# Vanlightly/vsr-tlaplus

Measured on AMD Instinct MI355X. Metric: distinct states/sec (whole node) + time-to-first-violation, VSR 3-replica, higher is better.
Workload: dtype u64

## Files before the change

vsr_tlaplus_amd/csrc/vsr_deep.hpp:

```cpp
#pragma once

namespace {

typedef DeepLevelRec DeepLevel;

struct Slicer {
  u64 cap_n, cap_w, g1, stride;
  u64 cap_c = ~(u64)0;
  double yield_n = 0, yield_w = 0;
  u64 worst() const {
    const u64 sz = std::min<u64>(std::min<u64>(cap_n / (4 * g1), cap_w / (4 * g1 * stride)), cap_c);
    return std::max<u64>(128, sz & ~(u64)127);
  }
  u64 next() const {
    if (yield_n <= 0) return worst();
    const double sz = std::min((double)cap_n / (3.0 * std::max(yield_n, 1e-3)), (double)cap_w / (3.0 * std::max(yield_w, 1e-3)));
    return std::max<u64>(worst(), std::min<u64>(cap_c, std::max<u64>(128, (u64)std::min(sz, 1e15) & ~(u64)127)));
  }
  void expect(double per_n, double per_w) { yield_n = std::max(yield_n, per_n); yield_w = std::max(yield_w, per_w); }
  void observe(u64 n_src, u64 n_out, u64 w_out) {
    if (!n_src) return;
    yield_n = std::max(yield_n, (double)n_out / (double)n_src);
    yield_w = std::max(yield_w, (double)w_out / (double)n_src);
  }
};

struct DeepRun;
struct DeepIo {
  void* ctx = nullptr;
  int world = 1;
  u64 cand_cap = 0;
  int (*pass)(void* ctx, const u64* sw, const u64* so, u64 n, u64 p_off, int level, int mode, u64 bag, const PassDst* dst) = nullptr;
  int (*any)(void* ctx, u64* flag) = nullptr;
  int (*reduce)(void* ctx, DeepRun* R) = nullptr;
  int (*resolve)(void* ctx, DeepRun* R) = nullptr;
};

struct DeepRun {
  vsrmc_checker* c;
  const DeepIo* io = nullptr;
  int base;
  int last_regen;
  bool insert;
  vsrmc_level_info ins, prb;
  u64 viol_ins = ~(u64)0;
  u32 mask_ins = 0, mask_prb = 0;
  std::vector<u64> bad;
  u64 launches = 0, n_slices = 0, n_subs = 0;
  u64* d_sum = nullptr;
  bool rebase = false;
  u64* d_cnt = nullptr;
  u32* d_err = nullptr;
  int err = 0;
  int probed_level() const { return last_regen + (insert ? 2 : 1); }
};

void deep_free_scratch(vsrmc_checker* c) {
  for (PassDst& B : c->scratch) {
    if (B.words && B.own_words) (void)hipFree(B.words);
    if (B.off && B.own_index) (void)hipFree(B.off);
    if (B.fp && B.own_index) (void)hipFree(B.fp);
  }
  c->scratch.clear();
  c->scratch0 = PassDst();
  c->scratch_carved = false;
  c->scratch_buf = -1;
  c->scratch_front = 0;
}

int deep_plan_scratch(vsrmc_checker* c, int count, bool carve = true, u64 front = 0) {
  if (count < 0) count = 0;
  if (count > 400) return fail(VSRMC_E_REP, "deep search: more than 400 nested levels");
  const int nxt = c->cur ^ 1;
  if ((c->host_frontier >> nxt) & 1) carve = false;
  front = (front + 63) & ~(u64)63;
  const bool same_buf = !c->scratch_carved || c->scratch_buf == nxt;
  if ((size_t)count <= c->scratch.size() && c->scratch_front == front && same_buf && (c->scratch_carved == carve || (count == 0 && !carve))) return 0;
  deep_free_scratch(c);
  if (count == 0) return 0;
  size_t free_b = 0, total_b = 0;
  HIPCHK(hipMemGetInfo(&free_b, &total_b));
  const char* share_env = std::getenv("VSRMC_AUTOSIZE_SHARE");
  const double share = share_env ? std::max(1.0, std::atof(share_env)) : 1.0;
  const double reserve = std::max(0.0, (double)free_b - 1.0e9) / share;
  if (front >= c->words_cap(nxt)) carve = false;
  const double idle_w = (double)(c->words_cap(nxt) - (carve ? front : 0));
  const int with0 = front ? 0 : 1;
  const u64 floor_w = (u64)1 << 21;
  const double w_old = std::max((double)floor_w, std::min(idle_w / 4.0, reserve / (double)count / 9.34));
  const double cost_old = (with0 ? 1.0 / idle_w : 0.0) + (double)count / w_old;
  int best_n = 0;
  double best_s = 0;
  if (carve)
    for (int n_idle = 1; n_idle <= count + with0; n_idle++) {
      const double from_res = (double)(count + with0 - n_idle) * 9.34 + (double)(n_idle - with0) * 1.34;
      const double s = std::min(idle_w / (double)n_idle, from_res > 0 ? reserve / from_res : 1e30);
      if (s > best_s) { best_s = s; best_n = n_idle; }
    }
  const bool carved = carve && best_n >= 1 + with0 && best_s >= (double)floor_w && (double)(count + with0) / best_s < cost_old;
  const u64 wcap = carved ? (u64)best_s & ~(u64)63 : (u64)w_old;
  auto alloc_index = [&](PassDst& B) -> bool {
    B.cap = std::max<u64>((u64)1 << 15, B.words_cap / 12);
    return hipMalloc((void**)&B.off, (B.cap + 1) * 8) == hipSuccess && hipMalloc((void**)&B.fp, B.cap * 8) == hipSuccess;
  };
  bool ok = true;
  if (carved && with0) {
    c->scratch0.words = c->words[nxt]; c->scratch0.words_cap = wcap; c->scratch0.own_words = false;
    c->scratch0.off = c->off[nxt]; c->scratch0.fp = c->lvl_fp; c->scratch0.own_index = false;
    c->scratch0.cap = std::min<u64>(c->opt.frontier_states, std::max<u64>((u64)1 << 15, wcap / 12));
  }
  for (int k = 1; k <= count && ok; k++) {
    PassDst B;
    B.words_cap = wcap;
    if (carved && k - 1 + with0 < best_n) { B.words = c->words[nxt] + front + (u64)(k - 1 + with0) * wcap; B.own_words = false; }
    else ok = hipMalloc((void**)&B.words, B.words_cap * 8) == hipSuccess;
    ok = ok && alloc_index(B);
    c->scratch.push_back(B);
  }
  if (!ok) {
    (void)hipGetLastError();
    deep_free_scratch(c);
    return fail(VSRMC_E_HIP, "hipMalloc of a deep-search scratch buffer failed");
  }
  c->scratch_carved = carve;
  c->scratch_buf = nxt;
  c->scratch_front = front;
  return 0;
}

int deep_buffer(vsrmc_checker* c, int k, PassDst* out) {
  const int nxt = c->cur ^ 1;
  if (k == 0) {
    if (c->scratch0.words) { *out = c->scratch0; return 0; }
    out->words = c->words[nxt]; out->words_cap = c->words_cap(nxt); out->off = c->off[nxt]; out->fp = c->lvl_fp; out->cap = c->opt.frontier_states;
    return 0;
  }
  if ((size_t)k > c->scratch.size()) return fail(VSRMC_E_REP, "deep search: a nesting level without a planned scratch buffer");
  *out = c->scratch[(size_t)k - 1];
  return 0;
}

void deep_acc(vsrmc_level_info* t, const LevelCtl& h, double ms) {
  t->generated += h.generated;
  t->deadlocks += h.deadlocks;
  t->probes += h.probes;
  for (int a = 0; a < 16; a++) t->act_generated[a] += h.act_generated[a];
  t->expand_ms += ms;
}

int deep_run_pass(DeepRun& R, const u64* sw, const u64* so, u64 n, u64 p_off, int level, int mode, u64 bag, const PassDst* dst) {
  R.c->extra_launches = 0;
  if (R.io) return R.io->pass(R.io->ctx, sw, so, n, p_off, level, mode, bag, dst);
  return expand_pass(R.c, sw, so, n, p_off, level, mode, bag, dst);
}

void deep_claim_bits_alloc(vsrmc_checker* c, u64 src_max_bag) {
  if (c->claim_bits) { (void)hipFree(c->claim_bits); c->claim_bits = nullptr; }
  c->claim_w = c->claim_parents = 0;
  if (c->opt.world > 1 || !c->regen_bits_kernel || !c->insert_kernel) return;
  const Model& M = c->model.M;
  const u64 ords = (u64)M.m0 + std::min<u64>(src_max_bag, (u64)M.max_bag) * (u64)(M.R + 1) + 1;
  const u64 w = (ords + 31) / 32, bytes = c->n_frontier * w * 4;
  if (w > 8) return;
  size_t free_b = 0, total_b = 0;
  if (hipMemGetInfo(&free_b, &total_b) != hipSuccess || (double)bytes > 0.4 * (double)free_b) return;
  if (hipMalloc((void**)&c->claim_bits, std::max<u64>(bytes, 4)) != hipSuccess) { (void)hipGetLastError(); c->claim_bits = nullptr; return; }
  if (hipMemsetAsync(c->claim_bits, 0, std::max<u64>(bytes, 4), c->stream) != hipSuccess) { (void)hipFree(c->claim_bits); c->claim_bits = nullptr; return; }
  c->claim_w = w;
  c->claim_parents = c->n_frontier;
}
bool deep_more(DeepRun& R, bool mine, int* rc) {
  u64 f = (mine ? 1 : 0) | (R.err ? 2 : 0);
  if (R.io) *rc = R.io->any(R.io->ctx, &f);
  if (!*rc && f >= 2) *rc = R.err ? R.err : fail(VSRMC_E_STATE, "deep pass: another rank failed between two exchanges");
  return !*rc && (f & 1) != 0;
}
int deep_local_fail(DeepRun& R, int rc) {
  if (!R.io) return rc;
  if (!R.err) R.err = rc;
  return 0;
}
u64 deep_cand_bound(const DeepRun& R, u64 g1) {
  if (!R.io || R.io->world <= 1) return ~(u64)0;
  return std::max<u64>(128, (u64)(0.45 * (double)R.io->cand_cap * (double)R.io->world / (double)std::max<u64>(1, g1)) & ~(u64)127);
}

int deep_probe(DeepRun& R, const PassDst& B, u64 n, int lv, u64 bag) {
  vsrmc_checker* c = R.c;
  if (!n) return 0;
  c->expand_ms = 0;
  if (R.err) return 0;
  int rc = expand_pass(c, B.words, B.off, n, 0, lv + 1, MODE_PROBE, bag);
  R.launches += c->extra_launches;
  if (!rc && c->h.limit_unchecked) {
    R.prb.limit_rechecked += c->h.limit_unchecked;
    c->probe_all_actions = true;
    rc = expand_pass(c, B.words, B.off, n, 0, lv + 1, MODE_PROBE, bag);
    c->probe_all_actions = false;
    R.launches += 1 + c->extra_launches;
  }
  if (rc) return deep_local_fail(R, rc);
  R.launches++;
  deep_acc(&R.prb, c->h, c->expand_ms);
  if (c->h.n_pending) {
    R.mask_prb |= c->h.viol_mask;
    if (c->h.n_pending > c->opt.pending_entries || R.bad.size() / 2 + c->h.n_pending > ((u64)1 << 24))
      return deep_local_fail(R, fail(VSRMC_E_REP, "more violating successors in the probed level than the pending list holds (pending_entries)"));
    const size_t at = R.bad.size();
    R.bad.resize(at + 2 * c->h.n_pending);
    if (hipMemcpy(R.bad.data() + at, c->pending, 16 * c->h.n_pending, hipMemcpyDeviceToHost) != hipSuccess)
      return deep_local_fail(R, fail(VSRMC_E_HIP, "deep search: copy of the probe's candidates"));
  }
  return 0;
}

int deep_export(DeepRun& R, const PassDst& B, u64 part) {
  vsrmc_checker* c = R.c;
  if (!part) return 0;
  const int nxt = c->cur ^ 1;
  hipLaunchKernelGGL(k_export, dim3((unsigned)((part + 63) / 64)), dim3(64), 0, c->stream, (const u64*)B.words, B.off, B.fp, (u64)0, part,
                     c->words[nxt], c->scratch_front ? c->scratch_front : c->words_cap(nxt), c->off[nxt], c->lvl_fp, c->opt.frontier_states, R.d_cnt, R.d_err);
  if (hipGetLastError() != hipSuccess || hipStreamSynchronize(c->stream) != hipSuccess) return fail(VSRMC_E_HIP, "deep search: k_export (re-basing)");
  return 0;
}

int deep_descend(DeepRun& R, const u64* src_words, const u64* src_off, u64 n_idx, u64 src_bag, int lv, int k) {
  vsrmc_checker* c = R.c;
  const Model& M = c->model.M;
  PassDst B;
  int rc = deep_buffer(c, k, &B);
  if (rc) return rc;
  Slicer sl;
  sl.cap_n = B.cap; sl.cap_w = B.words_cap; sl.g1 = std::max<u64>(1, c->deep_g); sl.stride = (u64)c->lds_stride;
  sl.cap_c = deep_cand_bound(R, sl.g1);
  const bool regen = lv + 1 <= R.last_regen;
  const DeepLevel& next = c->deep_lv[(size_t)(lv - R.base)];
  if (regen) {
    const u64 parents = lv == R.base ? c->n_valid : c->deep_lv[(size_t)(lv - R.base - 1)].n_local;
    const double per_n = (double)next.n_local / (double)std::max<u64>(1, parents);
    const double wbar = (lv == R.base ? (double)c->cur_w / (double)std::max<u64>(1, c->n_valid) : (double)(M.fixed + (int)src_bag)) + 2.0;
    sl.expect(per_n, per_n * wbar);
  }
  const u64 out_bag = regen ? std::min<u64>(next.max_bag, (u64)M.max_bag) : 0;
  for (u64 a = 0; deep_more(R, a < n_idx, &rc);) {
    if (rc) return rc;
    const u64 n = a < n_idx ? std::min<u64>(sl.next(), n_idx - a) : 0;
    c->expand_ms = 0;
    rc = deep_run_pass(R, src_words, src_off + a, n, (R.io && c->opt.world > 1) ? 0 : a, lv + 1, regen ? MODE_REGEN : MODE_NORMAL, src_bag, &B);
    if (rc) return rc;
    if (n) R.launches += 1 + c->extra_launches;
    a += n;
    if (n) (k == 0 ? R.n_slices : R.n_subs)++;
    const u64 part = c->h.n_new;
    sl.observe(n, part, c->h.words_new);
    if (regen) {
      R.ins.materialize_ms += c->expand_ms;
      if (lv + 1 == R.last_regen && !R.insert) rc = R.rebase ? deep_export(R, B, part) : deep_probe(R, B, part, lv + 1, out_bag);
      else rc = deep_descend(R, B.words, B.off, part, out_bag, lv + 1, k + 1);
      if (rc) return rc;
      continue;
    }
    deep_acc(&R.ins, c->h, c->expand_ms);
    R.ins.record_words += c->h.rec_words;
    R.ins.max_bag = std::max<u64>(R.ins.max_bag, c->h.max_bag);
    if (c->h.viol_fp != ~(u64)0) {
      R.mask_ins |= c->h.viol_mask;
      R.viol_ins = std::min<u64>(R.viol_ins, c->h.viol_fp);
    }
    if (!part) continue;
    const u64 bag_new = std::min<u64>(c->h.max_bag, (u64)M.max_bag);
    {
      u64 hsum[3] = {0, 0, 0};
      bool ok = hipMemsetAsync(R.d_sum, 0, 24, c->stream) == hipSuccess;
      if (ok) hipLaunchKernelGGL(k_level_checksum, dim3(1024), dim3(256), 0, c->stream, B.fp, part, R.d_sum);
      ok = ok && hipGetLastError() == hipSuccess && hipMemcpyAsync(hsum, R.d_sum, 24, hipMemcpyDeviceToHost, c->stream) == hipSuccess &&
           hipStreamSynchronize(c->stream) == hipSuccess;
      if (!ok) {
        rc = deep_local_fail(R, fail(VSRMC_E_HIP, "deep search: k_level_checksum"));
        if (rc) return rc;
        continue;
      }
      R.ins.fp_xor ^= hsum[0];
      R.ins.fp_sum += hsum[1];
      R.ins.n_new += hsum[2];
    }
    if (R.viol_ins != ~(u64)0) continue;
    rc = deep_probe(R, B, part, lv + 1, bag_new);
    if (rc) return rc;
  }
  return rc;
}

int deep_resolve(DeepRun& R) {
  vsrmc_checker* c = R.c;
  const u64 nbad = R.bad.size() / 2;
  if (!nbad) return 0;
  const int plevel = R.probed_level();
  std::vector<std::pair<u64, u64>> pairs(nbad);
  for (u64 i = 0; i < nbad; i++) pairs[i] = std::make_pair(R.bad[2 * i], R.bad[2 * i + 1]);
  std::sort(pairs.begin(), pairs.end());
  std::vector<u64> fps;
  for (u64 i = 0; i < nbad; i++)
    if (i == 0 || pairs[i].first != pairs[i - 1].first) fps.push_back(pairs[i].first);
  std::vector<uint8_t> seen8(fps.size(), 0);
  int rc = vsrmc_checker_seen_batch(c, fps.data(), (u64)fps.size(), plevel, seen8.data());
  if (rc) return rc;
  u64 first = ~(u64)0, key = ~(u64)0;
  size_t g = 0;
  for (u64 i = 0; i < nbad; i++) {
    if (i && pairs[i].first != pairs[i - 1].first) g++;
    if (seen8[g]) continue;
    R.prb.pending++;
    if (first == ~(u64)0) { first = pairs[i].first; key = pairs[i].second; }
    if (c->probe_viol.empty() || c->probe_viol.back() != pairs[i].first) {
      c->probe_viol.push_back(pairs[i].first);
      c->probe_viol_key.push_back(pairs[i].second);
    }
  }
  c->probe_viol_level = plevel;
  if (first == ~(u64)0) return 0;
  int found = 0;
  u64 pfp = 0, pmeta = 0;
  rc = table_lookup(c, meta_pfp(key), plevel - 1, 1, &found, &pfp, &pmeta);
  if (rc) return rc;
  if (found > 1) return fail(VSRMC_E_STATE, "ambiguous predecessor pointer: several states of the parent's level share the 45 fingerprint bits the violating successor keeps of its parent");
  R.prb.viol_fp = first;
  R.prb.viol_mask = (int32_t)R.mask_prb;
  if (found) { c->probe_fp = pfp; c->probe_level = plevel - 1; c->probe_extra_fp = first; }
  return 0;
}

int deep_check_ready(vsrmc_checker* c, int extra_levels, bool sharded) {
  if (c->opt.exact_ties) return fail(VSRMC_E_STATE, "levels beyond the record buffers need a single-pass checker");
  if (!sharded && c->opt.world > 1) return fail(VSRMC_E_STATE, "a sharded checker goes beyond its record buffers with vsrmc_shard_loop_deepen");
  if (c->failed) return fail(VSRMC_E_STATE, "the checker stopped on an error");
  if (c->level + c->deep + extra_levels >= 511) return fail(VSRMC_E_REP, "more than 510 BFS levels");
  return 0;
}

int deep_first_pass(vsrmc_checker* c, vsrmc_level_info* ins, const DeepIo* io = nullptr) {
  const Model& M = c->model.M;
  DeepRun R;
  R.c = c; R.io = io; R.base = c->level; R.last_regen = c->level; R.insert = true;
  std::memset(&R.ins, 0, sizeof(R.ins));
  std::memset(&R.prb, 0, sizeof(R.prb));
  R.ins.viol_fp = R.ins.viol_index = R.prb.viol_fp = R.prb.viol_index = ~(u64)0;
  const double t0 = now_s();
  const u64 bagL = c->bag_known ? c->cur_max_bag : (u64)M.max_bag;
  c->deep = 1;
  c->deep_lv.assign(1, DeepLevel());
  const u64 cb = deep_cand_bound(R, std::max<u64>(c->deep_g, c->g_last));
  if (!io || c->opt.world == 1) deep_claim_bits_alloc(c, bagL);
  int rc = 0;
  for (u64 a = 0; deep_more(R, a < c->n_frontier, &rc);) {
    if (rc) break;
    const u64 n = a < c->n_frontier ? std::min<u64>(cb, c->n_frontier - a) : 0;
    c->expand_ms = 0;
    rc = deep_run_pass(R, c->words[c->cur], c->off[c->cur] + a, n, (io && c->opt.world > 1) ? 0 : a, c->level + 1, MODE_INSERT, bagL, nullptr);
    if (rc) break;
    a += n;
    if (n) R.launches += 1 + c->extra_launches;
    deep_acc(&R.ins, c->h, c->expand_ms);
    R.ins.n_new += c->h.n_new;
    R.ins.max_bag = std::max<u64>(R.ins.max_bag, c->h.max_bag);
    R.ins.fp_xor ^= c->h.fp_xor;
    R.ins.fp_sum += c->h.fp_sum;
    if (c->h.viol_fp != ~(u64)0) { R.mask_ins |= c->h.viol_mask; R.viol_ins = std::min<u64>(R.viol_ins, c->h.viol_fp); }
  }
  if (rc) { c->failed = 1; return rc; }
  const u64 n_local = R.ins.n_new, frontier_local = c->n_valid;
  R.ins.frontier = c->n_valid;
  R.ins.viol_fp = R.viol_ins;
  R.ins.viol_mask = (int32_t)R.mask_ins;
  if (io && (rc = io->reduce(io->ctx, &R)) != 0) { c->failed = 1; return rc; }
  DeepLevel& d = c->deep_lv[0];
  d.n_new = R.ins.n_new; d.n_local = n_local; d.generated = R.ins.generated; d.max_bag = R.ins.max_bag; d.frontier = R.ins.frontier;
  c->deep_g = std::max<u64>(c->deep_g, (R.ins.generated + R.ins.frontier - 1) / std::max<u64>(1, R.ins.frontier) + 1);
  (void)frontier_local;
  *ins = R.ins;
  ins->level = c->level + (R.ins.n_new ? 1 : 0);
  if (R.ins.n_new == 0) { c->deep = 0; c->deep_lv.clear(); }
  ins->pending = R.launches;
  c->deep_distinct = c->distinct + (io ? n_local : R.ins.n_new);
  c->deep_generated = c->total_generated + R.ins.generated;
  ins->distinct = c->deep_distinct;
  ins->total_generated = c->deep_generated;
  ins->seconds = now_s() - t0;
  ins->viol_index = ~(u64)0;
  if (ins->viol_fp != ~(u64)0) {
    c->probe_fp = ins->viol_fp;
    c->probe_level = c->level + 1;
    c->probe_extra_fp = 0;
  } else {
    ins->viol_mask = 0;
  }
  return 0;
}

int deep_pass(vsrmc_checker* c, int last_regen, bool insert, vsrmc_level_info* ins, vsrmc_level_info* prb, const DeepIo* io = nullptr) {
  const Model& M = c->model.M;
  DeepRun R;
  R.c = c; R.io = io; R.base = c->level; R.last_regen = last_regen; R.insert = insert;
  std::memset(&R.ins, 0, sizeof(R.ins));
  std::memset(&R.prb, 0, sizeof(R.prb));
  R.ins.viol_fp = R.ins.viol_index = R.prb.viol_fp = R.prb.viol_index = ~(u64)0;
  const double t0 = now_s();
  if (io && c->opt.world > 1) {
    c->wepoch++;
  } else if (c->deep_regen_done) {
    hipLaunchKernelGGL(k_table_untake, dim3(4096), dim3(256), 0, c->stream, c->table, c->tmask + 1, c->level + 1);
    HIPCHK(hipGetLastError());
    HIPCHK(hipStreamSynchronize(c->stream));
  }
  c->deep_regen_done = true;
  int rc = 0;
  if (hipMalloc((void**)&R.d_sum, 24) != hipSuccess) { (void)hipGetLastError(); R.d_sum = nullptr; rc = fail(VSRMC_E_HIP, "deep pass: hipMalloc of the checksum words"); }
  struct FreeSum { u64* p; ~FreeSum() { if (p) (void)hipFree(p); } } free_sum{R.d_sum};
  if (insert) { c->deep_lv.resize((size_t)(last_regen + 1 - c->level)); c->deep_lv.back() = DeepLevel(); }
  if (!rc) rc = deep_plan_scratch(c, last_regen - c->level - (insert ? 0 : 1));
  if (io) {
    u64 bad_plan = rc ? 1 : 0;
    const int arc = io->any(io->ctx, &bad_plan);
    if (!rc && (arc || bad_plan)) rc = arc ? arc : fail(VSRMC_E_HIP, "deep pass: another rank could not allocate its scratch buffers");
  }
  if (rc) { c->failed = 1; return rc; }
  if (io) { u64 sync = 0; rc = io->any(io->ctx, &sync); }
  if (!rc) rc = deep_descend(R, c->words[c->cur], c->off[c->cur], c->n_frontier, c->bag_known ? c->cur_max_bag : (u64)M.max_bag, c->level, 0);
  if (rc) { c->failed = 1; return rc; }
  const u64 n_local = R.ins.n_new;
  R.ins.viol_fp = R.viol_ins;
  R.ins.viol_mask = (int32_t)R.mask_ins;
  R.prb.viol_mask = (int32_t)R.mask_prb;
  if (io && (rc = io->reduce(io->ctx, &R)) != 0) { c->failed = 1; return rc; }
  const double dt = now_s() - t0;
  const DeepLevel& below = c->deep_lv[(size_t)(last_regen - c->level - 1)];
  if (insert) {
    DeepLevel& d = c->deep_lv.back();
    d.n_new = R.ins.n_new; d.n_local = n_local; d.generated = R.ins.generated; d.max_bag = R.ins.max_bag; d.frontier = below.n_new;
    c->deep_g = std::max<u64>(c->deep_g, (R.ins.generated + below.n_new - 1) / std::max<u64>(1, below.n_new) + 1);
    c->deep_distinct += io ? n_local : R.ins.n_new;
    c->deep_generated += R.ins.generated;
    *ins = R.ins;
    ins->level = last_regen + (R.ins.n_new ? 1 : 0);
    ins->frontier = below.n_new;
    ins->distinct = c->deep_distinct;
    ins->total_generated = c->deep_generated;
    ins->pending = R.launches;
    ins->words_new = (R.n_slices << 32) | (R.n_subs & 0xFFFFFFFFull);
    ins->viol_index = ~(u64)0;
    const double ms_all = R.ins.expand_ms + R.ins.materialize_ms + R.prb.expand_ms;
    ins->seconds = dt * ((R.ins.expand_ms + R.ins.materialize_ms) / std::max(1e-9, ms_all));
    if (R.ins.n_new) c->deep = last_regen + 1 - c->level;
    else c->deep_lv.pop_back();
    if (ins->viol_fp != ~(u64)0) {
      c->probe_fp = ins->viol_fp;
      c->probe_level = last_regen + 1;
      c->probe_extra_fp = 0;
      return 0;
    }
    ins->viol_mask = 0;
  }
  R.prb.level = R.probed_level();
  R.prb.frontier = insert ? R.ins.n_new : below.n_new;
  R.prb.distinct = c->deep_distinct;
  R.prb.total_generated = c->deep_generated + R.prb.generated;
  R.prb.seconds = insert ? dt - ins->seconds : dt;
  R.prb.viol_fp = R.prb.viol_index = ~(u64)0;
  R.prb.viol_mask = 0;
  if (!insert) {
    R.prb.record_words = R.ins.record_words;
    R.prb.materialize_ms = R.ins.materialize_ms;
    R.prb.words_new = (R.n_slices << 32) | (R.n_subs & 0xFFFFFFFFull);
  }
  rc = io ? io->resolve(io->ctx, &R) : deep_resolve(R);
  if (rc) return rc;
  *prb = R.prb;
  return 0;
}

bool rebase_pays(const vsrmc_checker* c) {
  if (!c->deep || c->failed || c->opt.world > 1 || c->opt.exact_ties || c->rebase_off) return false;
  const DeepLevel& top = c->deep_lv.back();
  if (top.n_new == 0) return false;
  if (!(c->deep >= 2 || top.n_new <= c->n_valid)) return false;
  const Model& M = c->model.M;
  const int nxt = c->cur ^ 1;
  const double words = (double)top.n_new * (double)(M.fixed + (int)std::min<u64>(top.max_bag, (u64)M.max_bag));
  return words <= 0.8 * (double)c->words_cap(nxt) && (double)top.n_new <= 0.8 * (double)c->opt.frontier_states;
}

int deep_rebase(vsrmc_checker* c, vsrmc_level_info* out) {
  const Model& M = c->model.M;
  const int K = c->level + c->deep;
  DeepRun R;
  R.c = c; R.base = c->level; R.last_regen = K; R.insert = false; R.rebase = true;
  std::memset(&R.ins, 0, sizeof(R.ins));
  std::memset(&R.prb, 0, sizeof(R.prb));
  R.ins.viol_fp = R.ins.viol_index = R.prb.viol_fp = R.prb.viol_index = ~(u64)0;
  const double t0 = now_s();
  const u64 front_w = c->deep_lv.back().n_new * (u64)(M.fixed + (int)std::min<u64>(c->deep_lv.back().max_bag, (u64)M.max_bag));
  int rc = deep_plan_scratch(c, c->deep, true, front_w);
  if (rc) { c->rebase_off = true; return 1; }
  struct FreeCnt { u64* p; u32* q; ~FreeCnt() { if (p) (void)hipFree(p); if (q) (void)hipFree(q); } } free_cnt{nullptr, nullptr};
  if (hipMalloc((void**)&R.d_cnt, 16) != hipSuccess) { (void)hipGetLastError(); R.d_cnt = nullptr; c->rebase_off = true; return 1; }
  free_cnt.p = R.d_cnt;
  if (hipMalloc((void**)&R.d_err, 4) != hipSuccess) { (void)hipGetLastError(); R.d_err = nullptr; c->rebase_off = true; return 1; }
  free_cnt.q = R.d_err;
  if (hipMemsetAsync(R.d_cnt, 0, 16, c->stream) != hipSuccess || hipMemsetAsync(R.d_err, 0, 4, c->stream) != hipSuccess) { (void)hipGetLastError(); c->rebase_off = true; return 1; }
  if (c->deep_regen_done) {
    hipLaunchKernelGGL(k_table_untake, dim3(4096), dim3(256), 0, c->stream, c->table, c->tmask + 1, c->level + 1);
    HIPCHK(hipGetLastError());
    HIPCHK(hipStreamSynchronize(c->stream));
  }
  c->deep_regen_done = true;
  rc = deep_descend(R, c->words[c->cur], c->off[c->cur], c->n_frontier, c->bag_known ? c->cur_max_bag : (u64)M.max_bag, c->level, 1);
  if (rc) { c->failed = 1; return rc; }
  u64 cnt[2] = {0, 0};
  u32 xerr = 0;
  HIPCHK(hipMemcpy(cnt, R.d_cnt, 16, hipMemcpyDeviceToHost));
  HIPCHK(hipMemcpy(&xerr, R.d_err, 4, hipMemcpyDeviceToHost));
  const DeepLevel top = c->deep_lv.back();
  if (xerr || cnt[0] != top.n_new) {
    c->failed = 1;
    return fail(xerr ? VSRMC_E_REP : VSRMC_E_STATE, xerr ? std::string("re-basing: the idle record buffer is too small for the level after all")
                : "re-basing: level " + std::to_string(K) + " has " + std::to_string((unsigned long long)top.n_new) + " states, the descent regenerated " +
                  std::to_string((unsigned long long)cnt[0]));
  }
  const u64 below = c->deep >= 2 ? c->deep_lv[c->deep_lv.size() - 2].n_new : c->n_valid;
  c->cur ^= 1;
  c->level = K;
  c->n_frontier = cnt[0];
  c->n_valid = cnt[0];
  c->cur_w = cnt[1];
  c->cur_rec_w = cnt[1];
  c->distinct = c->deep_distinct;
  c->total_generated = c->deep_generated;
  c->cur_max_bag = std::min<u64>(top.max_bag, (u64)M.max_bag);
  c->bag_known = true;
  c->hist_new[0] = below;
  c->hist_new[1] = top.n_new;
  c->g_last = (top.generated + std::max<u64>(1, top.frontier) - 1) / std::max<u64>(1, top.frontier) + 1;
  c->deep = 0;
  c->deep_lv.clear();
  if (c->claim_bits) { (void)hipFree(c->claim_bits); c->claim_bits = nullptr; c->claim_w = c->claim_parents = 0; }
  c->deep_regen_done = false;
  std::memset(out, 0, sizeof(*out));
  out->level = K;
  out->frontier = below;
  out->n_new = top.n_new;
  out->distinct = c->distinct;
  out->total_generated = c->total_generated;
  out->max_bag = top.max_bag;
  out->words_new = cnt[1];
  out->record_words = cnt[1];
  out->pending = R.launches;
  out->materialize_ms = R.ins.materialize_ms;
  out->seconds = now_s() - t0;
  out->viol_fp = out->viol_index = ~(u64)0;
  return 0;
}

}

extern "C" {

int32_t vsrmc_checker_deepen(vsrmc_checker* c, vsrmc_level_info* inserted, vsrmc_level_info* probed) {
  if (!c || !inserted || !probed) return fail(VSRMC_E_ARG, "NULL argument");
  int rc = deep_check_ready(c, 2, false);
  if (rc) return rc;
  HIPCHK(hipSetDevice(c->opt.device));
// ... 35 lines not shown
```

vsr_tlaplus_amd/csrc/vsr_kernels.hpp:

```cpp
#pragma once
#include <hip/hip_runtime.h>

#include "vsr_actions.hpp"
#include "vrst_actions.hpp"
#include "vras_actions.hpp"

namespace vsr {

template <int MODEL>
struct ModelOps;
template <>
struct ModelOps<0> {
  template <bool GUARD_ONLY, typename PTR>
  static VSR_HD bool gen_(const Model& M, PTR rec, int ord, Delta& D) { return gen<GUARD_ONLY>(M, rec, ord, D); }
  template <typename PTR>
  static VSR_HD u32 guard_pre(const Model& M, PTR rec, u64 hdr, const u64* Areg, int slot, int* kind0, int info) {
    return guard_slot_pre(M, rec, hdr, Areg, slot, kind0, info);
  }
  template <typename PTR>
  static VSR_HD u32 guard(const Model& M, PTR rec, int slot, int* kind0) { return guard_slot(M, rec, slot, kind0); }
  static VSR_HD int other_kind(int) { return A_SendGetState; }
  template <typename PTR>
  static VSR_HD void hash_child_(const Model& M, PTR rec, const Delta& D, u64* Hc) { hash_child(M, rec, D, Hc); }
  template <typename PTR>
// ... 1165 lines not shown
                             (unsigned long long)(key | META_TAKEN)) == key;
        src = ref >> 8;
        plen = (int)(ref & 255);
        if (plen > stride) plen = stride;
      }
    }
    if (!win) plen = 0;
    const u64 wmask = __ballot(win);
    const u64 c_1 = __builtin_readcyclecounter();
    cyc_fetch += c_1 - c_0;
    if (wmask == 0) continue;
    for (int w = 0; w < 64; w++) {
      const int n2 = 2 * __builtin_amdgcn_readlane(plen, w);
      if (n2 == 0) continue;
      const u32* g = (const u32*)(fr_words + readlane64(src, w));
      __attribute__((address_space(3))) void* l = (__attribute__((address_space(3))) void*)(s_slot + w * stride);
      if (lane < n2) __builtin_amdgcn_global_load_lds((const __attribute__((address_space(1))) void*)(g + lane), l, 4, 0, 0);
      if (lane + 64 < n2) __builtin_amdgcn_global_load_lds((const __attribute__((address_space(1))) void*)(g + lane), l, 4, 256, 0);
      if (lane + 128 < n2) __builtin_amdgcn_global_load_lds((const __attribute__((address_space(1))) void*)(g + lane), l, 4, 512, 0);
      if (lane + 192 < n2) __builtin_amdgcn_global_load_lds((const __attribute__((address_space(1))) void*)(g + lane), l, 4, 768, 0);
    }
    asm volatile("s_waitcnt vmcnt(0)" ::: "memory");
    lds_wave_sync();
    const u64 c_2 = __builtin_readcyclecounter();
    cyc_stage += c_2 - c_1;
    u64 fp = 0;
    int clen = 0, bad = 0, nbag = 0;
    if (win) {
      u64* rec = s_slot + lane * stride;
      Delta D;
      Ops::template gen_<false>(M, (const u64*)rec, origin_ord(origin), D);
      u64 Hc[6];
      Ops::hash_child_(M, (const u64*)rec, D, Hc);
      u32 ak;
      canonical_fp(M, D.hdr, Hc, &fp, &ak);
      bad = Ops::invariants(M, (const u64*)rec, D);
#ifdef VSRMC_TEST_HOOKS
      if (M.test_bad_mask && fp == M.test_bad_fp) bad |= (int)M.test_bad_mask;
#endif
      nbag = hdr_nmsg(D.hdr);
      clen = M.fixed + nbag;
      if (clen > stride) clen = stride;
      rec[0] = D.hdr;
      u64* pb = rec + 1 + (D.r - 1) * M.wpr;
      pb[0] = D.rep[0];
      if (M.wpr > 1) pb[1] = D.rep[1];
      if (M.wpr > 2) pb[2] = D.rep[2];
      if (M.wpr > 3) pb[3] = D.rep[3];
#pragma unroll
      for (int k = 0; k < 6; k++)
        if (k < M.np) rec[M.h0 + k] = Hc[k];
      int a = 0;
#pragma unroll
      for (int k = 0; k < VSR_NSLOT; k++)
        if ((D.used >> k) & 1) {
          if (D.pj(k) >= 0) rec[M.fixed + D.pj(k)] = D.pnew[k];
          else if (plen + a < stride) rec[plen + (a++)] = D.pnew[k];
        }
    }
    lds_wave_sync();
    const u64 c_3 = __builtin_readcyclecounter();
    cyc_gen += c_3 - c_2;
    const int nwin = __popcll(wmask);
    int incl = clen;
    for (int o = 1; o < 64; o <<= 1) {
      int t = __shfl_up(incl, o);
      if (lane >= o) incl += t;
    }
    const u32 total = (u32)__builtin_amdgcn_readlane(incl, 63);
    const u32 rank = (u32)__popcll(wmask & (((u64)1 << lane) - 1));
    u64 idx;
    bool overflow = false;
    if (idx_left < (u32)nwin) {
      u64 nb = 0;
      if (lane == 0) nb = atomicAdd((unsigned long long*)cnt_n, (unsigned long long)ichunk);
      nb = readlane64(nb, 0);
      if (nb + ichunk > nx_cap) overflow = true;
      idx = rank < idx_left ? idx_base + rank : nb + (rank - idx_left);
      idx_base = nb + ((u32)nwin - idx_left);
      idx_left = ichunk - ((u32)nwin - idx_left);
    } else {
      idx = idx_base + rank;
      idx_base += (u32)nwin;
      idx_left -= (u32)nwin;
    }
    if (w_left < total) {
      u64 nb = 0;
      if (lane == 0) nb = atomicAdd((unsigned long long*)cnt_w, (unsigned long long)wchunk);
      nb = readlane64(nb, 0);
      if (nb + wchunk > nx_words_cap) overflow = true;
      w_base = nb;
      w_left = wchunk;
    }
    const u64 dst = w_base + (u64)(incl - clen);
    rec_words += total;
    w_base += total;
    w_left -= total;
    if (overflow) {
      if (lane == 0) raise_error(ctl, ERR_FRONTIER_FULL, idx_base);
      idx_left = 0;
      w_left = 0;
      continue;
    }
    for (int g = 0; g < 64; g += VSR_MAT_GROUP) {
      if (((wmask >> g) & ((1u << VSR_MAT_GROUP) - 1)) == 0) continue;
#pragma unroll
      for (int q = 0; q < VSR_MAT_GROUP; q++) {
        const u64 d = readlane64(dst, g + q);
        const int n = __builtin_amdgcn_readlane(clen, g + q);
        if (lane < n) nx_words[d + lane] = s_slot[(g + q) * stride + lane];
        if (lane + 64 < n) nx_words[d + lane + 64] = s_slot[(g + q) * stride + lane + 64];
      }
    }
    if (win) {
      nx_off[idx] = (dst << 8) | (u64)clen;
      lvl_fp[idx] = fp;
      if (bad) {
        atomicMin((unsigned long long*)&ctl->viol_fp, (unsigned long long)fp);
        atomicOr(&ctl->viol_mask, (u32)bad);
      }
    }
    int mb = nbag;
    for (int o = 32; o > 0; o >>= 1) {
      int t = __shfl_down(mb, o);
      mb = t > mb ? t : mb;
    }
    if (lane == 0 && (u64)mb > __hip_atomic_load(&ctl->max_bag, __ATOMIC_RELAXED, __HIP_MEMORY_SCOPE_AGENT))
      atomicMax((unsigned long long*)&ctl->max_bag, (unsigned long long)mb);
    lds_wave_sync();
    cyc_write += __builtin_readcyclecounter() - c_3;
  }
  if (lane == 0) {
    atomicAdd((unsigned long long*)&ctl->phase_cycles[5], (unsigned long long)(cyc_fetch + cyc_stage));
    atomicAdd((unsigned long long*)&ctl->phase_cycles[6], (unsigned long long)cyc_gen);
    atomicAdd((unsigned long long*)&ctl->phase_cycles[7], (unsigned long long)cyc_write);
    atomicAdd((unsigned long long*)&ctl->rec_words, (unsigned long long)rec_words);
  }
  for (u32 k = lane; k < idx_left; k += 64) {
    nx_off[idx_base + k] = 0;
    lvl_fp[idx_base + k] = 0;
  }
}

__global__ void k_count_valid(const u64* __restrict__ refs, u64 n, u64* out) {
  u64 i = (u64)blockIdx.x * blockDim.x + threadIdx.x;
  const u64 stride = (u64)gridDim.x * blockDim.x;
  u32 c = 0;
  for (; i < n; i += stride) c += refs[i] != 0 ? 1 : 0;
  for (int o = 32; o > 0; o >>= 1) c += __shfl_down(c, o);
  if ((threadIdx.x & 63) == 0 && c) atomicAdd((unsigned long long*)out, (unsigned long long)c);
}

__global__ void k_level_checksum(const u64* __restrict__ fps, u64 n, u64* out) {
  u64 i = (u64)blockIdx.x * blockDim.x + threadIdx.x;
  const u64 stride = (u64)gridDim.x * blockDim.x;
  u64 x = 0, s = 0, c = 0;
  for (; i < n; i += stride) {
    const u64 f = fps[i];
    x ^= f;
    s += f;
    c += f != 0 ? 1 : 0;
  }
  for (int o = 32; o > 0; o >>= 1) {
    x ^= __shfl_down(x, o);
    s += __shfl_down(s, o);
    c += __shfl_down(c, o);
  }
  if ((threadIdx.x & 63) == 0) {
    if (x) atomicXor((unsigned long long*)&out[0], (unsigned long long)x);
    if (s) atomicAdd((unsigned long long*)&out[1], (unsigned long long)s);
    if (c) atomicAdd((unsigned long long*)&out[2], (unsigned long long)c);
  }
}

__global__ void k_table_level_checksum(const Slot* __restrict__ table, u64 n_slots, int level, u64* out) {
  u64 i = (u64)blockIdx.x * blockDim.x + threadIdx.x;
  const u64 stride = (u64)gridDim.x * blockDim.x;
  u64 x = 0, s = 0, c = 0;
  for (; i < n_slots; i += stride) {
    const u64 f = table[i].fp;
    if (f != 0 && meta_level(table[i].meta) == level) { x ^= f; s += f; c++; }
  }
  for (int o = 32; o > 0; o >>= 1) {
    x ^= __shfl_down(x, o);
    s += __shfl_down(s, o);
    c += __shfl_down(c, o);
  }
  if ((threadIdx.x & 63) == 0 && c) {
    atomicXor((unsigned long long*)&out[0], (unsigned long long)x);
    atomicAdd((unsigned long long*)&out[1], (unsigned long long)s);
    atomicAdd((unsigned long long*)&out[2], (unsigned long long)c);
  }
}

__global__ void k_table_rehash(const Slot* __restrict__ old_table, u64 n_old, Slot* table, u64 tmask, u32* err) {
  u64 i = (u64)blockIdx.x * blockDim.x + threadIdx.x;
  const u64 stride = (u64)gridDim.x * blockDim.x;
  for (; i < n_old; i += stride) {
    const Slot s = old_table[i];
    if (s.fp == 0) continue;
    u32 np = 0;
    const Probe p = probe_insert(table, tmask, s.fp, CntReg{&np});
    if (p.full) { atomicExch(err, (u32)ERR_TABLE_FULL); continue; }
    table[p.slot].meta = s.meta;
  }
}

__global__ void k_wset_rehash(const u64* __restrict__ old_fp, const u32* __restrict__ old_epoch, u64 n_old, u64* fp, u32* epoch, u64 mask, u32* err) {
  u64 i = (u64)blockIdx.x * blockDim.x + threadIdx.x;
  const u64 stride = (u64)gridDim.x * blockDim.x;
  for (; i < n_old; i += stride) {
    const u64 f = old_fp[i];
    if (f == 0) continue;
    u64 j = wset_home(f, mask);
    bool done = false;
    for (u64 step = 0; step <= mask && step < 65536 && !done; step++, j = (j + 1) & mask)
      if (atomicCAS((unsigned long long*)&fp[j], 0ull, (unsigned long long)f) == 0) { epoch[j] = old_epoch[i]; done = true; }
    if (!done) atomicExch(err, (u32)ERR_TABLE_FULL);
  }
}

__global__ void k_table_untake(Slot* table, u64 n_slots, int min_level) {
  u64 i = (u64)blockIdx.x * blockDim.x + threadIdx.x;
  const u64 stride = (u64)gridDim.x * blockDim.x;
  for (; i < n_slots; i += stride) {
    const u64 m = table[i].meta;
    if (table[i].fp != 0 && (m & META_TAKEN) && m != META_EMPTY && meta_level(m) >= min_level) table[i].meta = m & ~META_TAKEN;
  }
}

__global__ void k_table_init(Slot* table, u64 slots) {
  for (u64 i = (u64)blockIdx.x * blockDim.x + threadIdx.x; i < slots; i += (u64)gridDim.x * blockDim.x) {
    table[i].fp = 0;
    table[i].meta = META_EMPTY;
  }
}

__global__ void k_claim_batch(Slot* table, u64 tmask, const u64* __restrict__ entries, u64 n, int level, u64* rslot,
                              LevelCtl* ctl) {
  u64 i = (u64)blockIdx.x * blockDim.x + threadIdx.x;
  if (i >= n) return;
  bool found_old, full;
  u32 np = 0;
  u64 slot = table_claim(table, tmask, entries[2 * i], entries[2 * i + 1], level, &found_old, CntReg{&np}, &full);
  if (full) raise_error(ctl, ERR_TABLE_FULL, entries[2 * i]);
  rslot[i] = found_old ? ~(u64)0 : slot;
  atomicAdd((unsigned long long*)&ctl->probes, (unsigned long long)np);
}
__global__ void k_verdict(Slot* table, const u64* __restrict__ entries, const u64* __restrict__ rslot, u64 n, uint8_t* verdict) {
  u64 i = (u64)blockIdx.x * blockDim.x + threadIdx.x;
  if (i >= n) return;
  u64 s = rslot[i];
  const u64 key = entries[2 * i + 1];
  verdict[i] = (s != ~(u64)0 && atomicCAS((unsigned long long*)&table[s].meta, (unsigned long long)key,
                                          (unsigned long long)(key | META_TAKEN)) == key) ? 1 : 0;
}
__global__ void k_claim_batch_fused(Slot* table, u64 tmask, const u64* __restrict__ entries, u64 n, int level, uint8_t* verdict,
                                    LevelCtl* ctl) {
  u64 i = (u64)blockIdx.x * blockDim.x + threadIdx.x;
  if (i >= n) return;
  const u64 fp = entries[2 * i], key = entries[2 * i + 1];
  if (fp == 0) {
    verdict[i] = 0;
    return;
  }
  bool claimed, full;
  u64 prev_meta;
  u32 np = 0;
  table_claim_fused(table, tmask, fp, key, level, &claimed, &prev_meta, CntReg{&np}, &full);
  if (full) raise_error(ctl, ERR_TABLE_FULL, fp);
  verdict[i] = claimed ? 1 : 0;
  if (prev_meta != META_EMPTY && meta_level(prev_meta) == level && meta_auxkey(prev_meta) != meta_auxkey(key))
    atomicAdd((unsigned long long*)&ctl->ties, 1ull);
  for (int o = 32; o > 0; o >>= 1) np += __shfl_down(np, o);
  if ((threadIdx.x & 63) == 0 && np) atomicAdd((unsigned long long*)&ctl->probes, (unsigned long long)np);
}
__global__ void k_apply_verdict(const u64* __restrict__ entries, const u64* __restrict__ cand_idx, const uint8_t* __restrict__ verdict,
                                u64 n, u64* nx_off, u64* lvl_fp, LevelCtl* ctl, const WSet* wset , int level) {
  u64 i = (u64)blockIdx.x * blockDim.x + threadIdx.x;
  if (i >= n) return;
  const u64 fp = entries[2 * i];
  if (fp == 0) return;
  const u64 e = cand_idx[i];
  const u64 idx = cand_index(e);
  if (verdict[i]) {
    if (wset && !wset_insert(wset, fp, level)) raise_error(ctl, ERR_TABLE_FULL, fp);
    const u32 bad = cand_bad(e);
    if (bad) {
      atomicMin((unsigned long long*)&ctl->viol_fp, (unsigned long long)fp);
      atomicOr(&ctl->viol_mask, bad);
    }
  } else {
    nx_off[idx] = 0;
    lvl_fp[idx] = 0;
  }
}
__device__ __forceinline__ u64 find_exact(const Slot* table, u64 tmask, u64 fp);
__global__ void k_count_verdict(const u64* __restrict__ entries, const u64* __restrict__ cand_idx, const uint8_t* __restrict__ verdict, u64 n,
                                u64* pending, u64 pending_cap, LevelCtl* ctl, const WSet* wset, int level) {
  u64 i = (u64)blockIdx.x * blockDim.x + threadIdx.x;
  u64 cnt = 0, fx = 0, fs = 0, bag = 0;
  if (i < n && entries[2 * i] != 0 && verdict[i]) {
    const u64 fp = entries[2 * i], e = cand_idx[i];
    if (wset && !wset_insert(wset, fp, level)) raise_error(ctl, ERR_TABLE_FULL, fp);
    cnt = 1; fx = fp; fs = fp; bag = cand_index(e);
    const u32 bad = cand_bad(e);
    if (bad) {
      const u64 k = atomicAdd((unsigned long long*)&ctl->n_pending, 1ull);
      if (k < pending_cap) { pending[2 * k] = fp; pending[2 * k + 1] = entries[2 * i + 1]; }
      atomicMin((unsigned long long*)&ctl->viol_fp, (unsigned long long)fp);
      atomicOr(&ctl->viol_mask, bad);
    }
  }
  for (int o = 32; o > 0; o >>= 1) {
    cnt += __shfl_down(cnt, o);
    fx ^= __shfl_down(fx, o);
    fs += __shfl_down(fs, o);
    const u64 t = __shfl_down(bag, o);
    bag = t > bag ? t : bag;
  }
  if ((threadIdx.x & 63) == 0 && cnt) {
// ... 490 lines not shown
```

Before: 1.833 billion.

## Overlap level checksum readback with next probe and vectorize checksum kernel

The per-slice checksum result is now copied into pinned host memory without a blocking stream sync whenever the next probe runs locally. The totals are accumulated after deep_probe, which is expected to synchronize the stream itself. This removes one host-device round trip per slice. The checksum kernel also switches to 128-bit vector loads with an 8x unroll and a block-level shared-memory reduction, cutting the number of global atomics. The deferred accumulation relies on deep_probe having synchronized the stream before the host reads the pinned buffer.

```diff
diff --git a/vsr_tlaplus_amd/csrc/vsr_deep.hpp b/vsr_tlaplus_amd/csrc/vsr_deep.hpp
--- a/vsr_tlaplus_amd/csrc/vsr_deep.hpp
+++ b/vsr_tlaplus_amd/csrc/vsr_deep.hpp
@@ -48,6 +48,7 @@
   std::vector<u64> bad;
   u64 launches = 0, n_slices = 0, n_subs = 0;
   u64* d_sum = nullptr;
+  u64* h_sum = nullptr;
   bool rebase = false;
   u64* d_cnt = nullptr;
   u32* d_err = nullptr;
@@ -269,24 +270,27 @@
     }
     if (!part) continue;
     const u64 bag_new = std::min<u64>(c->h.max_bag, (u64)M.max_bag);
-    {
-      u64 hsum[3] = {0, 0, 0};
-      bool ok = hipMemsetAsync(R.d_sum, 0, 24, c->stream) == hipSuccess;
-      if (ok) hipLaunchKernelGGL(k_level_checksum, dim3(1024), dim3(256), 0, c->stream, B.fp, part, R.d_sum);
-      ok = ok && hipGetLastError() == hipSuccess && hipMemcpyAsync(hsum, R.d_sum, 24, hipMemcpyDeviceToHost, c->stream) == hipSuccess &&
-           hipStreamSynchronize(c->stream) == hipSuccess;
-      if (!ok) {
-        rc = deep_local_fail(R, fail(VSRMC_E_HIP, "deep search: k_level_checksum"));
-        if (rc) return rc;
-        continue;
-      }
-      R.ins.fp_xor ^= hsum[0];
-      R.ins.fp_sum += hsum[1];
-      R.ins.n_new += hsum[2];
+    const bool probe_next = R.viol_ins == ~(u64)0;
+    const bool wait_now = !probe_next || R.io || !R.h_sum;
+    u64 hsum_now[3] = {0, 0, 0};
+    u64* const hsum = R.h_sum ? R.h_sum : hsum_now;
+    bool ok = hipMemsetAsync(R.d_sum, 0, 24, c->stream) == hipSuccess;
+    if (ok) hipLaunchKernelGGL(k_level_checksum, dim3(1024), dim3(256), 0, c->stream, B.fp, part, R.d_sum);
+    ok = ok && hipGetLastError() == hipSuccess && hipMemcpyAsync(hsum, R.d_sum, 24, hipMemcpyDeviceToHost, c->stream) == hipSuccess &&
+         (!wait_now || hipStreamSynchronize(c->stream) == hipSuccess);
+    if (!ok) {
+      (void)hipStreamSynchronize(c->stream);
+      rc = deep_local_fail(R, fail(VSRMC_E_HIP, "deep search: k_level_checksum"));
+      if (rc) return rc;
+      continue;
     }
-    if (R.viol_ins != ~(u64)0) continue;
-    rc = deep_probe(R, B, part, lv + 1, bag_new);
-    if (rc) return rc;
+    if (probe_next) {
+      rc = deep_probe(R, B, part, lv + 1, bag_new);
+      if (rc) return rc;
+    }
+    R.ins.fp_xor ^= hsum[0];
+    R.ins.fp_sum += hsum[1];
+    R.ins.n_new += hsum[2];
   }
   return rc;
 }
@@ -415,7 +419,8 @@
   c->deep_regen_done = true;
   int rc = 0;
   if (hipMalloc((void**)&R.d_sum, 24) != hipSuccess) { (void)hipGetLastError(); R.d_sum = nullptr; rc = fail(VSRMC_E_HIP, "deep pass: hipMalloc of the checksum words"); }
-  struct FreeSum { u64* p; ~FreeSum() { if (p) (void)hipFree(p); } } free_sum{R.d_sum};
+  if (hipHostMalloc((void**)&R.h_sum, 24) != hipSuccess) { (void)hipGetLastError(); R.h_sum = nullptr; }
+  struct FreeSum { u64* p; u64* h; ~FreeSum() { if (p) (void)hipFree(p); if (h) (void)hipHostFree(h); } } free_sum{R.d_sum, R.h_sum};
   if (insert) { c->deep_lv.resize((size_t)(last_regen + 1 - c->level)); c->deep_lv.back() = DeepLevel(); }
   if (!rc) rc = deep_plan_scratch(c, last_regen - c->level - (insert ? 0 : 1));
   if (io) {
diff --git a/vsr_tlaplus_amd/csrc/vsr_kernels.hpp b/vsr_tlaplus_amd/csrc/vsr_kernels.hpp
--- a/vsr_tlaplus_amd/csrc/vsr_kernels.hpp
+++ b/vsr_tlaplus_amd/csrc/vsr_kernels.hpp
@@ -1341,21 +1341,35 @@
 }
 
 __global__ void k_level_checksum(const u64* __restrict__ fps, u64 n, u64* out) {
-  u64 i = (u64)blockIdx.x * blockDim.x + threadIdx.x;
-  const u64 stride = (u64)gridDim.x * blockDim.x;
+  __shared__ u64 s_red[3][16];
+  const u64 t = (u64)blockIdx.x * blockDim.x + threadIdx.x, T = (u64)gridDim.x * blockDim.x;
+  const u64 head = n && (((uintptr_t)fps >> 3) & 1) ? 1 : 0;
+  const ulonglong2* __restrict__ v = (const ulonglong2*)(fps + head);
+  const u64 nvec = (n - head) >> 1;
   u64 x = 0, s = 0, c = 0;
-  for (; i < n; i += stride) {
-    const u64 f = fps[i];
-    x ^= f;
-    s += f;
-    c += f != 0 ? 1 : 0;
+  auto add = [&](u64 f) { x ^= f; s += f; c += f != 0 ? 1 : 0; };
+  for (u64 i = t; i < nvec; i += 8 * T) {
+    ulonglong2 a[8];
+#pragma unroll
+    for (int k = 0; k < 8; k++) a[k] = i + (u64)k * T < nvec ? v[i + (u64)k * T] : make_ulonglong2(0, 0);
+#pragma unroll
+    for (int k = 0; k < 8; k++) { add(a[k].x); add(a[k].y); }
+  }
+  if (t == 0) {
+    if (head) add(fps[0]);
+    if ((n - head) & 1) add(fps[n - 1]);
   }
   for (int o = 32; o > 0; o >>= 1) {
     x ^= __shfl_down(x, o);
     s += __shfl_down(s, o);
     c += __shfl_down(c, o);
   }
-  if ((threadIdx.x & 63) == 0) {
+  const int wave = threadIdx.x >> 6, nw = (blockDim.x + 63) >> 6;
+  if ((threadIdx.x & 63) == 0) { s_red[0][wave] = x; s_red[1][wave] = s; s_red[2][wave] = c; }
+  __syncthreads();
+  if (threadIdx.x == 0) {
+    x = s = c = 0;
+    for (int w = 0; w < nw; w++) { x ^= s_red[0][w]; s += s_red[1][w]; c += s_red[2][w]; }
     if (x) atomicXor((unsigned long long*)&out[0], (unsigned long long)x);
     if (s) atomicAdd((unsigned long long*)&out[1], (unsigned long long)s);
     if (c) atomicAdd((unsigned long long*)&out[2], (unsigned long long)c);
```

Result: no change. 1.845 billion, median of 6 (+0.6%).
